# ninocarrillo/pymodem

Hardware: AMD Instinct MI355X
Metric: Msamples/s through demod_chain (higher is better)
Workload: dtype f64+i8

## Files before the change

### include/pymodem_amd.h

```cpp
#ifndef PYMODEM_AMD_H
#define PYMODEM_AMD_H

#include <stddef.h>
#include <stdint.h>

#ifdef __cplusplus
extern "C" {
#endif

#define PM_VERSION 100

typedef enum pm_status {
    PM_OK = 0,
    PM_ERR_HIP = -1,
    PM_ERR_ARG = -2,
    PM_ERR_NODEV = -3,
    PM_ERR_CAPACITY = -4,
    PM_ERR_NOCONVERGE = -5
} pm_status;

typedef struct pm_ctx pm_ctx;

int pm_version(void);
int pm_device_count(void);
// ... 381 lines not shown
    double ms_to_demod_done, ms_to_sliced, ms_to_done;
    double done_at_ms;
} pm_pipe_result;
typedef struct pm_pipe pm_pipe;
int pm_pipe_create(pm_ctx *ctx, const pm_pipe_desc *desc, pm_pipe **out);
int pm_pipe_submit(pm_pipe *pipe, const int16_t *d_audio, int64_t n, int64_t *h_ticket);
int pm_pipe_submit_many(pm_pipe *pipe, const int16_t *const *d_audio, const int64_t *n, int count, int64_t *h_first_ticket);
int pm_pipe_promise(pm_pipe *pipe, int count, int64_t *h_first_ticket);
int pm_pipe_wait(pm_pipe *pipe, int64_t ticket, pm_pipe_result *out);
int pm_pipe_slices(pm_pipe *pipe, int64_t ticket, int chain, const uint8_t **h_data, const int64_t **h_addr, const uint8_t **h_plain, int64_t *h_count);
int pm_pipe_bitmap(pm_pipe *pipe, int64_t ticket, int chain, uint64_t *h_words, int64_t words);
int pm_pipe_slots(pm_pipe *pipe);
int pm_pipe_release(pm_pipe *pipe, int64_t ticket);
int pm_pipe_drain(pm_pipe *pipe);
int pm_pipe_stats(pm_pipe *pipe, int64_t *h_batches, int64_t *h_batch_recordings, double *h_slice_busy_ms, double *h_host_busy_ms);
pm_ctx *pm_pipe_side_ctx(pm_pipe *pipe, int worker);
pm_ctx *pm_pipe_demod_ctx(pm_pipe *pipe, int k);
int pm_pipe_destroy(pm_pipe *pipe);

#ifdef __cplusplus
}
#endif
#endif
```

### pymodem_amd/_native.py

```python
import ctypes
import os

_HERE = os.path.dirname(os.path.abspath(__file__))
_LIB = None


class NativeError(RuntimeError):
    pass


def library_path():
    return os.environ.get("PYMODEM_AMD_LIB") or os.path.join(_HERE, "libpymodem_amd.so")


class AGCParams(ctypes.Structure):
    _fields_ = [(k, ctypes.c_double) for k in ("attack_rate", "decay_rate", "sustain_time", "sample_rate", "target_amplitude")]


class Loop(ctypes.Structure):
    _fields_ = [(k, ctypes.c_double) for k in (
        "phase_scaling", "index_scaling", "set_frequency", "b0", "b1", "a1", "p_rate", "i_rate", "i_limit", "gain",
        "phase", "control", "sine", "cosine", "x0", "x1", "y0", "integral", "proportional",
        "bb0", "bb1", "ba1", "cx0", "cx1", "cy0", "sx0", "sx1", "sy0")]

# ... 270 lines not shown
    "pm_lbatch_tail_ctx": ([_vp], _vp),
    "pm_lbatch_loop_ctx": ([_vp], _vp),
    "pm_lbatch_slice_ctx": ([_vp], _vp),
    "pm_lbatch_destroy": ([_vp], _int),
    "pm_prof_intervals": ([_vp, _int, _vp, _vp, _i64, ctypes.POINTER(_i64)], _int),
    "pm_pipe_create": ([_vp, ctypes.POINTER(PipeDesc), ctypes.POINTER(_vp)], _int),
    "pm_pipe_submit": ([_vp, _vp, _i64, ctypes.POINTER(_i64)], _int),
    "pm_pipe_submit_many": ([_vp, _vp, _vp, _int, _vp], _int),
    "pm_pipe_promise": ([_vp, _int, _vp], _int),
    "pm_pipe_wait": ([_vp, _i64, ctypes.POINTER(PipeResult)], _int),
    "pm_pipe_release": ([_vp, _i64], _int),
    "pm_pipe_slices": ([_vp, _i64, _int, ctypes.POINTER(_vp), ctypes.POINTER(_vp), ctypes.POINTER(_vp), ctypes.POINTER(_i64)], _int),
    "pm_pipe_bitmap": ([_vp, _i64, _int, _vp, _i64], _int),
    "pm_pipe_slots": ([_vp], _int),
    "pm_pipe_drain": ([_vp], _int),
    "pm_pipe_stats": ([_vp, ctypes.POINTER(_i64), ctypes.POINTER(_i64), ctypes.POINTER(ctypes.c_double), ctypes.POINTER(ctypes.c_double)], _int),
    "pm_pipe_side_ctx": ([_vp, _int], _vp),
    "pm_pipe_demod_ctx": ([_vp, _int], _vp),
    "pm_pipe_destroy": ([_vp], _int),
    "pm_costas_bpsk": ([_vp, ctypes.POINTER(Loop), _int, _vp, _vp, _i64, _i64, _vp, _i64], _int),
    "pm_costas_qpsk": ([_vp, ctypes.POINTER(Loop), _int, _vp, _vp, _i64, _i64, _vp, _vp, _i64], _int),
    "pm_pll_afsk": ([_vp, ctypes.POINTER(Loop), _int, _vp, _vp, _i64, _i64, _vp, _i64], _int),
    "pm_mpsk_loop": ([_vp, ctypes.POINTER(Loop), _int, _vp, _vp, _vp, _vp, _i64, _i64, _vp, _vp, _i64], _int),
    "pm_slice_binary": ([_vp, _vp, _i64, ctypes.POINTER(SlicerParams), _vp, _vp, _i64, ctypes.POINTER(_i64)], _int),
    "pm_slice_quadrature": ([_vp, _vp, _vp, _i64, ctypes.POINTER(SlicerParams), _vp, _vp, _i64, ctypes.POINTER(_i64)], _int),
    "pm_slice_batch": ([_vp, ctypes.POINTER(SliceJob), _int], _int),
    "pm_slicer_tune": ([_vp, _i64], _int),
    "pm_slicer_limits": ([_vp, _i64], _int),
    "pm_slice_compact": ([_vp, _vp, _int, _vp, ctypes.c_size_t, ctypes.POINTER(_i64), ctypes.POINTER(ctypes.c_size_t)], _int),
    "pm_stream_scan": ([_vp, ctypes.POINTER(ScanJob), _int, _vp, ctypes.c_size_t, ctypes.POINTER(_i64), ctypes.POINTER(ctypes.c_size_t)], _int),
# ... 69 lines not shown
```

### pymodem_amd/chain_execute.py

```python
import ctypes
from concurrent.futures import ThreadPoolExecutor

import numpy as np

from ._native import Loop, check, lib, quick
from .device import Context, DeviceBuffer
from .modems import AFSKModem, AFSKPLLModem, BPSKModem, MPSKModem, QPSKModem
from .slicer import slice_batch


def process_chain(chain, input_audio):
    demod_audio = chain[1].demod(input_audio)
    sliced_data = chain[2].slice(demod_audio)
    descrambled_data = chain[3].stream_unscramble_8bit(sliced_data)
    return chain[4].decode(descrambled_data)


def multiprocess_chain(chain, input_audio, queue):
    queue.put(process_chain(chain, input_audio))


def process_chain_device(chain, input_audio, stages=None):
    demod_audio = chain[1].demod_signs(input_audio)
    sliced_data = chain[2].slice(demod_audio)
# ... 943 lines not shown
        check(lib().pm_pipe_bitmap(self._h, int(ticket), int(chain), buf.ctypes.data_as(ctypes.c_void_p), max(words, 1)))
        return np.unpackbits(buf.view(np.uint8), bitorder="little")[: int(nout)].astype(bool)

    def release(self, ticket):
        check(lib().pm_pipe_release(self._h, int(ticket)))

    def drain(self):
        check(lib().pm_pipe_drain(self._h))

    def stats(self):
        b, r = ctypes.c_int64(), ctypes.c_int64()
        s, h = ctypes.c_double(), ctypes.c_double()
        check(lib().pm_pipe_stats(self._h, ctypes.byref(b), ctypes.byref(r), ctypes.byref(s), ctypes.byref(h)))
        return {"slice_batches": b.value, "recordings": r.value, "slice_busy_ms": s.value, "host_busy_ms": h.value}

    def side_contexts(self):
        out = []
        for entry, first in ((lib().pm_pipe_side_ctx, 0), (lib().pm_pipe_demod_ctx, 1)):
            i = first
            while True:
                c = entry(self._h, i)
                if not c:
                    break
                out.append(Context.borrowed(c, self._ctx.device))
                i += 1
        return out

    def _destroy(self):
        h, self._h = self._h, None
        if h is not None:
# ... 95 lines not shown
```

### pymodem_amd/csrc/pm_afsk.hip

```cpp
#include "pm_fir_dev.h"
#include "pm_bpf8_dev.h"
#include "pm_afsk_sweep.h"
#include <chrono>
#include <cmath>
#include <cstdlib>
#include <cstring>

namespace {
using namespace pm_sweep;

template <int R, bool VEC, bool SPLIT = false>
__global__ __launch_bounds__(kThreads) void afsk_correlate_kernel(const double *__restrict__ x, int64_t n,
                                                                  const double *__restrict__ mi, const double *__restrict__ mq,
                                                                  const double *__restrict__ si, const double *__restrict__ sq,
                                                                  int m, double *__restrict__ y, int64_t nout, double *__restrict__ y2 = nullptr)
{
    extern __shared__ double xs[];
    constexpr int T = kThreads * R;
    const int t = threadIdx.x;
    const int span = T + m - 1;
    const int64_t tile0 = (int64_t)blockIdx.x * T;
    if (VEC) {
        stage_vec<R>(x, n, tile0, span, t, xs);
    } else {
// ... 161 lines not shown
    for (int i = 0; i < L; ++i) {
        mv[i] = slide_sqrt(a * a + b * b);
        sv[i] = slide_sqrt(c * c + d * d);
        if (i + 1 < L) {
            const double xk = xr[i], xn = xr[slide_slot<L>(i + m)];
            const double a2 = __builtin_fma(T.mr, a, __builtin_fma(-T.ms, b, __builtin_fma(-T.mer, xk, xn)));
            const double b2 = __builtin_fma(T.ms, a, __builtin_fma(T.mr, b, -T.mes * xk));
            const double c2 = __builtin_fma(T.sr, c, __builtin_fma(-T.ss, d, __builtin_fma(-T.ser, xk, xn)));
            const double d2 = __builtin_fma(T.ss, c, __builtin_fma(T.sr, d, -T.ses * xk));
            a = a2; b = b2; c = c2; d = d2;
        }
    }
}

typedef const double __attribute__((address_space(4))) *const_f64_ptr;
template <int L>
__device__ __forceinline__ void slide_run_f32(const double *__restrict__ xs, const double *__restrict__ tp, int run, int m, const SlideTones &T,
                                              float (&mv)[L], float (&sv)[L], const double *tg = nullptr)
{
    const double *xr = xs + run * (L + 1);
    double a = 0.0, b = 0.0, c = 0.0, d = 0.0;
    if (tg) {
        const_f64_ptr tq = (const_f64_ptr)tg;
        const double *xb = xr;
        int i = 0;
        for (; i + L <= m; i += L, xb += L + 1, tq += 4 * L) {
#pragma unroll
            for (int j = 0; j < L; ++j) {
                const double v = xb[j];
                a = __builtin_fma(tq[4 * j + 0], v, a);
                b = __builtin_fma(tq[4 * j + 1], v, b);
                c = __builtin_fma(tq[4 * j + 2], v, c);
                d = __builtin_fma(tq[4 * j + 3], v, d);
            }
        }
        for (int j = 0; i + j < m; ++j) {
            const double v = xb[j];
            a = __builtin_fma(tq[4 * j + 0], v, a);
            b = __builtin_fma(tq[4 * j + 1], v, b);
            c = __builtin_fma(tq[4 * j + 2], v, c);
            d = __builtin_fma(tq[4 * j + 3], v, d);
        }
    } else {
        const double2v *tq = reinterpret_cast<const double2v *>(tp);
        const double *xb = xr;
        int i = 0;
        for (; i + L <= m; i += L, xb += L + 1, tq += 2 * L) {
#pragma unroll
            for (int j = 0; j < L; ++j) {
                const double v = xb[j];
                const double2v h01 = tq[2 * j], h23 = tq[2 * j + 1];
                a = __builtin_fma(h01.x, v, a);
                b = __builtin_fma(h01.y, v, b);
                c = __builtin_fma(h23.x, v, c);
                d = __builtin_fma(h23.y, v, d);
            }
        }
        for (int j = 0; i + j < m; ++j) {
            const double v = xb[j];
            const double2v h01 = tq[2 * j], h23 = tq[2 * j + 1];
            a = __builtin_fma(h01.x, v, a);
            b = __builtin_fma(h01.y, v, b);
            c = __builtin_fma(h23.x, v, c);
            d = __builtin_fma(h23.y, v, d);
        }
    }
#pragma unroll
    for (int i = 0; i < L; ++i) {
        mv[i] = __builtin_amdgcn_sqrtf((float)__builtin_fma(a, a, b * b));
        sv[i] = __builtin_amdgcn_sqrtf((float)__builtin_fma(c, c, d * d));
        if (i + 1 < L) {
            const double xk = xr[i], xn = xr[slide_slot<L>(i + m)];
            const double a2 = __builtin_fma(T.mr, a, __builtin_fma(-T.ms, b, __builtin_fma(-T.mer, xk, xn)));
            const double b2 = __builtin_fma(T.ms, a, __builtin_fma(T.mr, b, -T.mes * xk));
            const double c2 = __builtin_fma(T.sr, c, __builtin_fma(-T.ss, d, __builtin_fma(-T.ser, xk, xn)));
            const double d2 = __builtin_fma(T.ss, c, __builtin_fma(T.sr, d, -T.ses * xk));
            a = a2; b = b2; c = c2; d = d2;
        }
    }
}

// ... 391 lines not shown
#define PM_LPF8_F32MAG 1
#endif

#ifndef PM_LPF8_RECOMB32
#define PM_LPF8_RECOMB32 1
#endif
#ifndef PM_LPF8_WAVES
#define PM_LPF8_WAVES 4
#endif
template <bool ONE>
__device__ __forceinline__ void lpf8_sweep_tile(double *__restrict__ xs, unsigned char *__restrict__ planes, double *__restrict__ tp, int4v *__restrict__ bl,
                                                unsigned *__restrict__ wl, float *__restrict__ wmax8, int sweep, bool lds_ok, int t, int64_t tile0,
                                                const double *__restrict__ mi, const double *__restrict__ mq, const double *__restrict__ ui,
                                                const double *__restrict__ uq, int m, const SlideTones &T, const Lpf8Args &Q, int ml, int64_t nout, int G,
                                                const SweepArgs &P, double E, unsigned long long *__restrict__ list, int *__restrict__ count, int cap,
                                                const double *tg = nullptr)
{
    constexpr int L = kFuseRun, TILE = kThreads * 8;
    const int nmag = TILE + ml - 1, nruns = (nmag + L - 1) / L;
    if (!tg)
        for (int i = t; i < m; i += kThreads) {
            tp[4 * i + 0] = mi[m - 1 - i];
            tp[4 * i + 1] = mq[m - 1 - i];
            tp[4 * i + 2] = ui[m - 1 - i];
            tp[4 * i + 3] = uq[m - 1 - i];
        }
    lds_barrier();
#if PM_LPF8_F32MAG
    float mv[L], sv[L];
    if (t < nruns) slide_run_f32<L>(xs, tp, t, m, T, mv, sv, tg);
    float vmaxf = 0.0f, vsumf = 0.0f;
    if (t < nruns) {
        if (ONE) {
            const float g0 = (float)P.gain[0], ag0 = fabsf(g0);
#pragma unroll
            for (int i = 0; i < L; ++i) {
                vsumf = fmaxf(vsumf, fmaf(ag0, sv[i], mv[i]));
                mv[i] = fmaf(-g0, sv[i], mv[i]);
            }
        }
#pragma unroll
        for (int i = 0; i < L; ++i) vmaxf = fmaxf(vmaxf, ONE ? fabsf(mv[i]) : fmaxf(mv[i], sv[i]));
    }
#pragma unroll
    for (int off = 32; off > 0; off >>= 1) {
// ... 62 lines not shown
                    const double sc = scalable ? __builtin_fma(val[4 * q + i], scale, 6755399441055744.0) : 6755399441055744.0;
                    w[i] = ((unsigned)__double2loint(sc) + 0x808080u) ^ 0x808080u;
#endif
                }
                const unsigned a01 = __builtin_amdgcn_perm(w[1], w[0], 0x05010400u), a23 = __builtin_amdgcn_perm(w[3], w[2], 0x05010400u);
                unsigned char *at = planes + (size_t)stream * kL8Dig * kL8Plane + L * t + 4 * q;
                *reinterpret_cast<unsigned *>(at) = __builtin_amdgcn_perm(a23, a01, 0x05040100u);
                *reinterpret_cast<unsigned *>(at + kL8Plane) = __builtin_amdgcn_perm(a23, a01, 0x07060302u);
                *reinterpret_cast<unsigned *>(at + 2 * kL8Plane) =
                    __builtin_amdgcn_perm(w[1], w[0], 0x0c0c0602u) | __builtin_amdgcn_perm(w[3], w[2], 0x06020c0cu);
            }
        };
        put(mv, 0);
        if (!ONE) put(sv, 1);
    }
    const int lane = t & 63, wave = t >> 6, r = lane & 15, g4 = lane >> 4;
    for (int i = t; i < 2 * kL8Dig * 64; i += kThreads) bl[i] = Q.btab[i];
    lds_barrier();
    const int64_t nout64 = ((nout + 63) >> 6) * 64;
#pragma unroll 1
    for (int q = 0; q < 2; ++q) {
        const int tl = (wave * 2 + q) * 256;
        const int64_t go = tile0 + tl;
        if (go >= nout64) break;
        double a[4], b[4];
#pragma unroll
        for (int stream = 0; stream < (ONE ? 1 : 2); ++stream) {
            int4v acc[kL8Acc];
#pragma unroll
            for (int w = 0; w < kL8Acc; ++w) acc[w] = int4v{0, 0, 0, 0};
// ... 47 lines not shown
            if (uns) {
#pragma unroll
                for (int v = 0; v < 4; ++v)
                    if (16 * v < lim && !(fabs(y[v]) > Ecmp)) {
                        const unsigned mine = lds_ok ? atomicAdd(&wl[kTailCap], 1u) : (unsigned)kTailCap;
                        if (mine < (unsigned)kTailCap) {
                            wl[mine] = ((unsigned)sweep << 20) | ((unsigned)g << 16) | (unsigned)(tl + 64 * g4 + 16 * v + r);
                        } else {
                            const int idx = atomicAdd(count, 1);
                            if (idx < cap) list[idx] = ((unsigned long long)g << 48) | (unsigned long long)(go + 64 * g4 + 16 * v + r);
                        }
                    }
            }
        }
    }
}

template <bool ONE>
__global__ __launch_bounds__(kThreads) __attribute__((amdgpu_waves_per_eu(PM_LPF8_WAVES, PM_LPF8_WAVES))) void afsk_slide_lpf8_kernel(const double *__restrict__ x, int64_t n, const double *__restrict__ mi,
                                                                   const double *__restrict__ mq, const double *__restrict__ ui,
                                                                   const double *__restrict__ uq, int m, SlideTones T, Lpf8Args Q, int ml,
                                                                   int64_t nout, int G, SweepArgs P, double E, unsigned long long *__restrict__ list,
                                                                   int *__restrict__ count, int cap, int region0, SweepTail TL)
{
    extern __shared__ double xs[];
    constexpr int L = kFuseRun, TILE = kThreads * 8;
    const int t = threadIdx.x;
    const int64_t tile0 = (int64_t)blockIdx.x * TILE;
    const int nmag = TILE + ml - 1, nruns = (nmag + L - 1) / L, xspan = nruns * L + m - 1;
    double *tp = xs + region0;
// ... 46 lines not shown
    unsigned long long *list;
    int *count;
    int64_t nout;
};
struct FusedArgs {
    FusedSweep s[2];
    const int16_t *audio;
    int64_t n, nb;
    const pm_bpf8_dev::i4 *bp_btab;
    pm_bpf8_dev::Scales sc;
    SweepSource src;
    int xs_span;
    int aplane;
    int xw_doubles, plane_bytes, mmax;
    int lds_ok, cap;
};

#ifndef PM_FUSED8_WAVES
#define PM_FUSED8_WAVES 5
#endif
template <int KB, bool ONE0, int NS, bool ONE1>
__global__ __launch_bounds__(kThreads) __attribute__((amdgpu_waves_per_eu(PM_FUSED8_WAVES, PM_FUSED8_WAVES))) void afsk_fused8_kernel(FusedArgs A)
{
    extern __shared__ double xs[];
#if defined(PM_FUSED8_PRIO) && PM_FUSED8_PRIO > 0
    __builtin_amdgcn_s_setprio(PM_FUSED8_PRIO);
#endif
    constexpr int L = kFuseRun, TILE = kThreads * 8;
    const int t = threadIdx.x, lane = t & 63, wave = t >> 6;
    const int64_t tile0 = (int64_t)blockIdx.x * TILE;
    unsigned char *const planes = reinterpret_cast<unsigned char *>(xs + A.xw_doubles);
    double *const tp = reinterpret_cast<double *>(planes + A.plane_bytes);
    int4v *const bl = reinterpret_cast<int4v *>(tp + 4 * A.mmax);
    unsigned *const wl = reinterpret_cast<unsigned *>(bl + 2 * kL8Dig * 64);
    float *const wmax8 = reinterpret_cast<float *>(wl + kTailCap + 4);
    if (t == 0) wl[kTailCap] = 0;
    unsigned char *const ap0 = planes, *const ap1 = planes + A.aplane;
    pm_bpf8_dev::stage_planes_rt(A.audio, A.n, tile0, t, kThreads, ap0, ap1, A.aplane);
    {
        lds_barrier();
        const int r = lane & 15, g = lane >> 4;
        const int ntiles = (A.xs_span + 255) >> 8;
        for (int q = wave; q < ntiles; q += kThreads / 64) {
            double val[4];
            const pm_bpf8_dev::i4 *bt = A.bp_btab;
            asm volatile("" : "+s"(bt));
            pm_bpf8_dev::tile_values_tab<KB, 4>(ap0, ap1, bt, q * 256, lane, A.sc, val);
#pragma unroll
            for (int v = 0; v < 4; ++v) {
                const int p = q * 256 + 16 * (4 * g + v) + r;
                if (p < A.xs_span) xs[slide_slot<L>(p)] = tile0 + p < A.nb ? val[v] : 0.0;
            }
        }
    }
    lds_barrier();
    {
        const FusedSweep &S = A.s[0];
        if (tile0 < ((S.nout + 63) >> 6) * 64)
            lpf8_sweep_tile<ONE0>(xs, planes, tp, bl, wl, wmax8, 0, A.lds_ok != 0, t, tile0, S.mi, S.mq, S.ui, S.uq, S.m, S.T, S.Q, S.ml, S.nout, S.G, S.P, S.E,
                                  S.list, S.count, A.cap, S.tg);
    }
    if (NS == 2) {
        lds_barrier();
        const FusedSweep &S = A.s[1];
        if (tile0 < ((S.nout + 63) >> 6) * 64)
            lpf8_sweep_tile<ONE1>(xs, planes, tp, bl, wl, wmax8, 1, A.lds_ok != 0, t, tile0, S.mi, S.mq, S.ui, S.uq, S.m, S.T, S.Q, S.ml, S.nout, S.G, S.P, S.E,
                                  S.list, S.count, A.cap, S.tg);
    }
    __syncthreads();
    const int ne = (int)(wl[kTailCap] < (unsigned)kTailCap ? wl[kTailCap] : (unsigned)kTailCap);
    for (int e = 0; e < ne; ++e) {
        const unsigned ent = wl[e];
        const int g = (int)(ent >> 16) & 15;
        const int64_t k = tile0 + (int64_t)(ent & 0xFFFFu);
        if (NS == 1 || (ent >> 20) == 0) {
            const FusedSweep &S = A.s[0];
            const double *si = S.space + (size_t)g * 2 * S.m;
            sweep_tail_entry<kThreads>(xs, t, nullptr, S.mi, S.mq, si, si + S.m, S.m, S.lpf, S.ml, A.src, k, reinterpret_cast<unsigned long long *>(S.P.bits[g]));
        } else {
            const FusedSweep &S = A.s[1];
            const double *si = S.space + (size_t)g * 2 * S.m;
            sweep_tail_entry<kThreads>(xs, t, nullptr, S.mi, S.mq, si, si + S.m, S.m, S.lpf, S.ml, A.src, k, reinterpret_cast<unsigned long long *>(S.P.bits[g]));
        }
    }
}

__global__ void sweep_mail_reset_kernel(int *__restrict__ count, int *__restrict__ keep, int *__restrict__ mail, int n)
{
    if ((int)threadIdx.x < n) {
        const int c = count[threadIdx.x];
        keep[threadIdx.x] = c;
        mail[threadIdx.x] = c;
        count[threadIdx.x] = 0;
    }
    __threadfence_system();
}

template <bool AUDIO>
__global__ __launch_bounds__(64) void sweep_exact_kernel(const double *__restrict__ x, const double *__restrict__ mi, const double *__restrict__ mq,
// ... 430 lines not shown
    int v = 0;
    PM_HIP(hipMemcpyAsync(&v, ctx->sweep_count, sizeof(int), hipMemcpyDeviceToHost, ctx->stream));
    PM_HIP(hipStreamSynchronize(ctx->stream));
    *h_uncertain = v;
    return PM_OK;
}

int pm_afsk_group_run(pm_ctx *ctx, const int16_t *d_audio, int64_t n, const double *d_bpf, int mb, double *d_bpf_out, double x_bound,
                      const pm_afsk_sweep_desc *h_sweeps, int nsweeps, int64_t *h_tickets)
{
    return pm_afsk_group_run_plan(ctx, d_audio, n, d_bpf, mb, d_bpf_out, x_bound, h_sweeps, nsweeps, h_tickets, nullptr, nullptr);
}

}

static int afsk_group_run_fused(pm_ctx *ctx, const int16_t *d_audio, int64_t n, const double *d_bpf, int mb, double x_bound, const pm_afsk_sweep_desc *h_sweeps,
                                int nsweeps, const pm_bpf8_plan *plan, const pm_lpf8_plan *const *lpf8, const pm_sweep_cells *cells, bool *fused)
{
    *fused = false;
    if (!plan || !lpf8 || !cells || !cells->d_list || nsweeps < 1 || nsweeps > 2 || ctx->tune.afsk_split || ctx->tune.afsk_unfused || ctx->tune.fuse_run == 16 ||
        ((uintptr_t)d_audio & 15) != 0)
        return PM_OK;
    int kb = 0;
    const void *btab = nullptr;
    double sc6[6];
    if (pm_bpf8_plan_view(plan, &kb, &btab, sc6) != PM_OK || (kb != 3 && kb != 4)) return PM_OK;
    FusedArgs A;
    memset(&A, 0, sizeof(A));
    const int64_t nb = n - mb + 1;
    const double e_x = pm_bpf8_error(plan);
    if (!(e_x >= 0.0 && e_x < 1e-6 * x_bound)) return PM_OK;
    SweepShape shape[2];
    for (int k = 0; k < nsweeps; ++k) shape[k] = SweepShape{h_sweeps[k].m, h_sweeps[k].ml, h_sweeps[k].groups == 1};
    const Lpf8Layout Y = lpf8_layout(shape, nsweeps, mb, kb);
    if (!Y.fuses) return PM_OK;
    for (int k = 0; k < nsweeps; ++k) {
        const pm_afsk_sweep_desc &w = h_sweeps[k];
        const pm_lpf8_plan *q = lpf8[k];
        if (!q || !w.h_tones || w.m < 2 || q->ml != w.ml || w.groups < 1 || w.groups > kSweepMax || !w.h_bits || !w.h_gains) return PM_OK;
        if (!(w.h_tones->tap_dev >= 0.0 && w.h_tones->tap_dev < 1e-6) || !(w.lpf_abs_sum > 0.0 && w.lpf_abs_sum < 1e300)) return PM_OK;
        if (nb < (int64_t)w.m + w.ml - 1) return PM_OK;
        FusedSweep &S = A.s[k];
        S.mi = w.d_mark_i; S.mq = w.d_mark_q; S.ui = w.d_unit_i; S.uq = w.d_unit_q;
        S.space = w.d_space; S.lpf = w.d_lpf;
        {
            pm_lpf8_plan *mq_ = const_cast<pm_lpf8_plan *>(q);
            if (!(mq_->d_tpl && mq_->tpl_m == w.m && mq_->tpl_src[0] == w.d_mark_i && mq_->tpl_src[1] == w.d_mark_q && mq_->tpl_src[2] == w.d_unit_i &&
                  mq_->tpl_src[3] == w.d_unit_q)) {
                if (mq_->d_tpl) { PM_HIP(hipStreamSynchronize(ctx->stream)); (void)hipFree(mq_->d_tpl); mq_->d_tpl = nullptr; }
                PM_HIP(hipMalloc(&mq_->d_tpl, sizeof(double) * 4 * (size_t)w.m + 256));
                hipLaunchKernelGGL(pack_templates_kernel, dim3((unsigned)pm_cdiv(4 * (int64_t)w.m, 256)), dim3(256), 0, ctx->stream, w.d_mark_i, w.d_mark_q, w.d_unit_i,
                                   w.d_unit_q, w.m, (double *)mq_->d_tpl);
                PM_HIP(hipGetLastError());
                PM_HIP(hipStreamSynchronize(ctx->stream));
                mq_->tpl_m = w.m;
                mq_->tpl_src[0] = w.d_mark_i; mq_->tpl_src[1] = w.d_mark_q; mq_->tpl_src[2] = w.d_unit_i; mq_->tpl_src[3] = w.d_unit_q;
            }
            S.tg = ctx->tune.sweep_lds_templates ? nullptr : (const double *)mq_->d_tpl;
        }
        S.m = w.m; S.ml = w.ml; S.G = w.groups;
        S.one = w.groups == 1;
        double gmax = 0.0;
        if (!sweep_args(w.h_gains, w.h_bits, w.groups, &S.P, &gmax)) return PM_OK;
        S.T = slide_tones(w.h_tones);
        S.E = sweep_bound(w.m, w.lpf_abs_sum, gmax, x_bound, w.h_tones, kFuseRun, e_x);
        S.Q = lpf8_args(q, gmax, S.one);
        S.list = cells->d_list + (size_t)k * kSweepCap;
        S.count = cells->d_count + k;
        S.nout = nb - w.m - w.ml + 2;
    }
    A.audio = d_audio;
    A.n = n;
    A.nb = nb;
    A.bp_btab = (const pm_bpf8_dev::i4 *)btab;
// ... 2 lines not shown
    A.src = SweepSource{d_audio, d_bpf, mb, e_x};
    A.xs_span = Y.xs_span; A.aplane = Y.aplane; A.mmax = Y.mmax;
    A.xw_doubles = Y.xw_doubles; A.plane_bytes = Y.plane_bytes;
    A.cap = kSweepCap;
    A.lds_ok = Y.lds_ok && !ctx->tune.sweep_no_tail;
    const size_t lds_launch = Y.lds + (size_t)std::max(0, ctx->tune.fused_lds_pad);
    int64_t tiles = 0;
    double bits_out = 0.0, flops = 2.0 * mb * (double)nb;
    for (int k = 0; k < nsweeps; ++k) {
        tiles = std::max(tiles, pm_cdiv(A.s[k].nout, (int64_t)kThreads * 8));
        bits_out += (double)A.s[k].G * (double)A.s[k].nout / 8;
        flops += (4.0 * A.s[k].m / kFuseRun + 18.0) * (double)(nb - A.s[k].m + 1) + (A.s[k].one ? 1.0 : 2.0) * 2.0 * A.s[k].ml * (double)A.s[k].nout +
                 2.0 * A.s[k].G * (double)A.s[k].nout;
    }
    PM_ARG(tiles >= 1 && tiles < (1LL << 31));
    {
        PmProf prof(ctx, PM_K_FIR_F64);
        prof.work((double)n * 2 + bits_out, flops);
        auto go = [&](auto kernel) -> int {
            if (int rc = allow_lds(kernel, lds_launch)) return rc;
            hipLaunchKernelGGL(kernel, dim3((unsigned)tiles), dim3(kThreads), lds_launch, ctx->stream, A);
            return PM_OK;
        };
        int rc = PM_OK;
        const bool o0 = A.s[0].one != 0, o1 = nsweeps == 2 && A.s[1].one != 0;
#define PM_FUSED_GO(KB)                                                                                                             \
        rc = nsweeps == 1 ? (o0 ? go(afsk_fused8_kernel<KB, true, 1, false>) : go(afsk_fused8_kernel<KB, false, 1, false>))              \
                          : (o0 ? (o1 ? go(afsk_fused8_kernel<KB, true, 2, true>) : go(afsk_fused8_kernel<KB, true, 2, false>))          \
                                : (o1 ? go(afsk_fused8_kernel<KB, false, 2, true>) : go(afsk_fused8_kernel<KB, false, 2, false>)));
        if (kb == 3) { PM_FUSED_GO(3) } else { PM_FUSED_GO(4) }
// ... 158 lines not shown
```

### pymodem_amd/csrc/pm_bpf8_dev.h

```cpp
#pragma once
#include <hip/hip_runtime.h>
#include <cstdint>

namespace pm_bpf8_dev {

typedef int i4 __attribute__((ext_vector_type(4)));

struct Scales { double s[5]; double c0; };

__device__ __forceinline__ void stage_planes_rt(const int16_t *__restrict__ x, int64_t n, int64_t wg0, int t, int threads, unsigned char *__restrict__ p0,
                                                unsigned char *__restrict__ p1, int span)
{
    for (int p = t * 8; p < span; p += threads * 8) {
        const int64_t gi = wg0 + p;
        uint32_t d0 = 0, d1 = 0, d2 = 0, d3 = 0;
        if (gi + 8 <= n) {
            const uint4 v = *reinterpret_cast<const uint4 *>(x + gi);
            d0 = v.x; d1 = v.y; d2 = v.z; d3 = v.w;
        } else {
            uint16_t s[8];
#pragma unroll
            for (int q = 0; q < 8; ++q) s[q] = gi + q < n ? (uint16_t)x[gi + q] : (uint16_t)0;
            d0 = s[0] | (uint32_t)s[1] << 16; d1 = s[2] | (uint32_t)s[3] << 16; d2 = s[4] | (uint32_t)s[5] << 16; d3 = s[6] | (uint32_t)s[7] << 16;
        }
// ... 51 lines not shown
#pragma unroll
        for (int b = 0; b < D; ++b) {
            acc[b] = __builtin_amdgcn_mfma_i32_16x16x64_i8(a0, B[b], acc[b], 0, 0, 0);
            acc[b + 1] = __builtin_amdgcn_mfma_i32_16x16x64_i8(a1, B[b], acc[b + 1], 0, 0, 0);
        }
    }
#pragma unroll
    for (int v = 0; v < 4; ++v) {
        double x = sc.c0;
#pragma unroll
        for (int w = 0; w < kWeights; ++w) x = __builtin_fma((double)acc[w][v], sc.s[w], x);
        val[v] = x;
    }
}

}
```

### pymodem_amd/csrc/pm_common.h

```cpp
#pragma once
#include <hip/hip_runtime.h>
#include <cstdarg>
#include <cstdint>
#include <cstdio>
#include <vector>
#include "../../include/pymodem_amd.h"

constexpr size_t PM_PINNED_BYTES = 256 * 1024;
constexpr int kSweepRing = 64;
constexpr int kSweepCap = 65536;

struct pm_sweep_cells {
    int *d_count = nullptr;
    int *h_mail = nullptr;
    unsigned long long *d_list = nullptr;
};

struct pm_tuning {
    int fir_no_short = 0;
    int fuse_run = 0;
    int afsk_unfused = 0;
    int afsk_lpf8 = 0;
    int loop_wide = -1;
    int64_t loop_lds_min = 0;
// ... 98 lines not shown
int pm_bpf8_rows_max(pm_ctx *ctx, const pm_bpf8_plan *p, const int16_t *const *d_rows, int rows, int64_t n, unsigned long long *d_keys, double *d_out,
                     unsigned long long *d_redone = nullptr);
struct pm_lpf8_plan {
    int ml = 0, S = 0, device = 0;
    double tapq_int = 0;
    double qabs = 0;
    double dlow = 0;
    double hmax = 0;
    void *d_btab = nullptr;
    void *d_tpl = nullptr;
    const void *tpl_src[4] = {nullptr, nullptr, nullptr, nullptr};
    int tpl_m = 0;
};
int pm_lpf8_plan_create(pm_ctx *ctx, const double *h_taps, int ml, pm_lpf8_plan **out);
void pm_lpf8_plan_destroy(pm_lpf8_plan *p);
int pm_afsk_group_run_plan(pm_ctx *ctx, const int16_t *d_audio, int64_t n, const double *d_bpf, int mb, double *d_bpf_out, double x_bound,
                           const pm_afsk_sweep_desc *h_sweeps, int nsweeps, int64_t *h_tickets, const pm_bpf8_plan *plan,
                           const pm_lpf8_plan *const *lpf8 = nullptr, const pm_sweep_cells *cells = nullptr);
int pm_afsk_sweep_exact_list(pm_ctx *ctx, const int16_t *d_audio, const double *d_bpf, int mb, const pm_afsk_sweep_desc *w, uint64_t *const *h_bits,
                             const unsigned long long *d_list, const int *d_count);

extern "C" int pm_codec_fetch_batch_clean(pm_codec *const *codecs, const int64_t *counts, int n, pm_packet *h_out, int threads);

struct pm_rowslice;
int pm_rowslice_create(pm_ctx *ctx, const pm_slicer_params *h_params, int chains, pm_rowslice **out);
void pm_rowslice_destroy(pm_rowslice *rs);
bool pm_rowslice_made_for(const pm_rowslice *rs, const pm_slicer_params *h_params, int chains);
int pm_rowslice_chunk(pm_ctx *ctx, const pm_rowslice *rs, int rows, int quad, const uint64_t *d_bi, const uint64_t *d_bq, int64_t stride, int64_t first,
                      int64_t count, pm_rowslice_rec *d_recs, uint8_t *d_data, uint16_t *d_steps, int64_t cap);

// ... 22 lines not shown
```

### pymodem_amd/csrc/pm_pipe.hip

```cpp
#include "pm_common.h"
#include <atomic>
#include <chrono>
#include <condition_variable>
#include <cstring>
#include <deque>
#include <map>
#include <memory>
#include <mutex>
#include <string>
#include <pthread.h>
#include <thread>
#include <vector>

namespace {

constexpr int kMaxChains = 64;
constexpr int kCompactHead = PM_COMPACT_HEAD;

double now_ms()
{
    return std::chrono::duration<double, std::milli>(std::chrono::steady_clock::now().time_since_epoch()).count();
}

struct HostBlock {
// ... 87 lines not shown
    unsigned long long *d_lists = nullptr;
    std::vector<int> free_cells;
    bool keep_slices = false, trace = false;
    bool packets = false;
    bool frames = false;
    bool addrs = false;
    bool scan = false;
    bool host_copy = false;
    bool skip_decode = false;
    int64_t next_ticket = 0, submitted = 0, finished = 0;
    int64_t promised = 0;
    bool promise_failed = false;
    bool closing = false;
    std::vector<std::thread> threads;
    std::atomic<int64_t> batches{0}, batch_recordings{0};
    double busy_slice_ms = 0, busy_host_ms = 0, t_origin = now_ms();
};

namespace {

void rows_clean(RowBlock *b)
{
    for (int64_t k = 0; k < b->used; ++k) {
        pm_packet &q = b->rows[k];
        const int32_t len = k < (int64_t)b->lens.size() ? b->lens[(size_t)k] : PM_PKT_MAX;
        memset(q.data, 0, (size_t)len);
        memset(&q, 0, offsetof(pm_packet, data));
    }
    b->used = 0;
    b->lens.clear();
// ... 162 lines not shown
                    p->slice_q.pop_front();
                }
                if (hipEventSynchronize(nxt->demod_done) != hipSuccess) fail(*nxt, pm_set_error(PM_ERR_HIP, "the demod stage of recording %lld failed", (long long)nxt->ticket));
                nxt->t_ready = now_ms();
                batch.push_back(nxt);
            }
        }
        const double t0 = now_ms();
        const int nch = p->nchains, nb = (int)batch.size();
        int rc = PM_OK;
        std::vector<int> cells_back;
        for (auto &r : batch) {
            if (!p->nsweeps) break;
            std::vector<int64_t> unc(p->nsweeps);
            for (int s = 0; s < p->nsweeps; ++s) unc[s] = ((volatile int *)p->h_cells)[(size_t)r->cell * p->nsweeps + s];
            for (int s = 0; s < p->nsweeps && !r->status; ++s) {
                if (unc[s] <= 0) continue;
                if (unc[s] <= kSweepCap) {
                    if ((rc = pm_afsk_sweep_exact_list(side, r->d_audio, p->d_bpf, p->mb, &p->sweeps[s], p->sweep_bits_store[r->slot][s].data(),
                                                       p->d_lists + ((size_t)r->cell * p->nsweeps + s) * kSweepCap, p->d_cells + (size_t)r->cell * 2 * p->nsweeps + p->nsweeps + s)))
                        fail(*r, rc);
                    continue;
                }
                for (int c = 0; c < nch && !r->status; ++c)
                    if (p->chains[c].sweep == s && (rc = exact_chain(p, side, w, *r, c))) fail(*r, rc);
            }
            cells_back.push_back(r->cell);
            r->cell = -1;
        }
        std::vector<std::pair<int, int>> act;
// ... 456 lines not shown
                if (hipMemcpy(h.data(), d.d_bpf, h.size() * sizeof(double), hipMemcpyDeviceToHost) != hipSuccess)
                    rc = pm_set_error(PM_ERR_HIP, "pm_pipe_create: reading the band-pass taps back failed");
                else
                    rc = pm_bpf8_plan_create(ctx, h.data(), d.mb, &p->bpf8);
            }
        }
        p->lpf8.assign(d.nsweeps, nullptr);
        {
            const char *e = getenv("PM_PIPE_LPF8");
            for (int s = 0; s < d.nsweeps && !rc && !(e && e[0] == '0'); ++s) {
                const pm_afsk_sweep_desc &w = p->sweeps[s];
                if (!p->has_tones[s] || w.ml + 15 > 128 || w.m < 2) continue;
                std::vector<double> h((size_t)w.ml);
                if (hipMemcpy(h.data(), w.d_lpf, h.size() * sizeof(double), hipMemcpyDeviceToHost) != hipSuccess)
                    rc = pm_set_error(PM_ERR_HIP, "pm_pipe_create: reading the low-pass taps back failed");
                else
                    rc = pm_lpf8_plan_create(ctx, h.data(), w.ml, &p->lpf8[s]);
            }
        }
        if (rc) break;
        p->bits_words = (size_t)(d.max_samples + 63) / 64 + 2;
        p->d_bits.assign((size_t)p->slots * d.nchains, nullptr);
        for (size_t i = 0; i < p->d_bits.size() && !rc; ++i) {
            if (!(rc = pm_malloc(ctx, p->bits_words * 8, &q))) p->d_bits[i] = (uint64_t *)q;
        }
        if (rc) break;
        p->sweep_bits_store.resize(p->slots);
        for (int sl = 0; sl < p->slots; ++sl) {
            p->sweep_bits_store[sl].resize(d.nsweeps);
            for (int s = 0; s < d.nsweeps; ++s) {
                p->sweep_bits_store[sl][s].resize(p->sweeps[s].groups);
                for (int g = 0; g < p->sweeps[s].groups; ++g) p->sweep_bits_store[sl][s][g] = p->d_bits[(size_t)sl * d.nchains + seen[s][g]];
// ... 256 lines not shown
    PM_HIP(hipMemcpy(h_words, p->d_bits[(size_t)slot * p->nchains + p->bit_owner[chain]], (size_t)words * 8, hipMemcpyDeviceToHost));
    return PM_OK;
}

int pm_pipe_stats(pm_pipe *p, int64_t *h_batches, int64_t *h_batch_recordings, double *h_slice_busy_ms, double *h_host_busy_ms)
{
    PM_ARG(p != nullptr);
    std::unique_lock<std::mutex> lk(p->mu);
    if (h_batches) *h_batches = p->batches.load();
    if (h_batch_recordings) *h_batch_recordings = p->batch_recordings.load();
    if (h_slice_busy_ms) *h_slice_busy_ms = p->busy_slice_ms;
    if (h_host_busy_ms) *h_host_busy_ms = p->busy_host_ms;
    return PM_OK;
}

pm_ctx *pm_pipe_side_ctx(pm_pipe *p, int worker)
{
    return (p && worker >= 0 && worker < (int)p->side.size()) ? p->side[worker] : nullptr;
}

pm_ctx *pm_pipe_demod_ctx(pm_pipe *p, int k)
{
    return (p && k >= 0 && k < (int)p->demod.size()) ? p->demod[k] : nullptr;
}

}
```

Measured before the change: 284,200.

## Software-pipeline template sums and band-pass MFMA operands, pack templates at pipe creation

The sliding start sums now go through a double-buffered fetch/compute helper that loads the next group of template taps and samples while FMAs run on the current group. The int8 band-pass MFMA loop prefetches the next k-block's weight operands into registers ahead of use. Template packing moves from the per-run fused launch path to pipe creation, which removes a possible allocation and stream sync from the hot path. The change also adds an optional s_memtime phase clock (compiled out by default) and a counter of mailed undecided cells. The prefetching uses more registers, which could lower occupancy.

```diff
diff --git a/include/pymodem_amd.h b/include/pymodem_amd.h
--- a/include/pymodem_amd.h
+++ b/include/pymodem_amd.h
@@ -419,6 +419,7 @@
 int pm_pipe_release(pm_pipe *pipe, int64_t ticket);
 int pm_pipe_drain(pm_pipe *pipe);
 int pm_pipe_stats(pm_pipe *pipe, int64_t *h_batches, int64_t *h_batch_recordings, double *h_slice_busy_ms, double *h_host_busy_ms);
+int pm_pipe_undecided(pm_pipe *pipe, int64_t *h_mailed);
 pm_ctx *pm_pipe_side_ctx(pm_pipe *pipe, int worker);
 pm_ctx *pm_pipe_demod_ctx(pm_pipe *pipe, int k);
 int pm_pipe_destroy(pm_pipe *pipe);
diff --git a/pymodem_amd/_native.py b/pymodem_amd/_native.py
--- a/pymodem_amd/_native.py
+++ b/pymodem_amd/_native.py
@@ -308,6 +308,7 @@
     "pm_pipe_bitmap": ([_vp, _i64, _int, _vp, _i64], _int),
     "pm_pipe_slots": ([_vp], _int),
     "pm_pipe_drain": ([_vp], _int),
+    "pm_pipe_undecided": ([_vp, ctypes.POINTER(_i64)], _int),
     "pm_pipe_stats": ([_vp, ctypes.POINTER(_i64), ctypes.POINTER(_i64), ctypes.POINTER(ctypes.c_double), ctypes.POINTER(ctypes.c_double)], _int),
     "pm_pipe_side_ctx": ([_vp, _int], _vp),
     "pm_pipe_demod_ctx": ([_vp, _int], _vp),
diff --git a/pymodem_amd/chain_execute.py b/pymodem_amd/chain_execute.py
--- a/pymodem_amd/chain_execute.py
+++ b/pymodem_amd/chain_execute.py
@@ -981,6 +981,11 @@
         check(lib().pm_pipe_stats(self._h, ctypes.byref(b), ctypes.byref(r), ctypes.byref(s), ctypes.byref(h)))
         return {"slice_batches": b.value, "recordings": r.value, "slice_busy_ms": s.value, "host_busy_ms": h.value}
 
+    def undecided(self):
+        k = ctypes.c_int64()
+        check(lib().pm_pipe_undecided(self._h, ctypes.byref(k)))
+        return k.value
+
     def side_contexts(self):
         out = []
         for entry, first in ((lib().pm_pipe_side_ctx, 0), (lib().pm_pipe_demod_ctx, 1)):
diff --git a/pymodem_amd/csrc/pm_afsk.hip b/pymodem_amd/csrc/pm_afsk.hip
--- a/pymodem_amd/csrc/pm_afsk.hip
+++ b/pymodem_amd/csrc/pm_afsk.hip
@@ -5,6 +5,7 @@
 #include <cmath>
 #include <cstdlib>
 #include <cstring>
+#include <mutex>
 
 namespace {
 using namespace pm_sweep;
@@ -199,57 +200,99 @@
 }
 
 typedef const double __attribute__((address_space(4))) *const_f64_ptr;
+
+enum { kPhStart, kPhStaged, kPhBandpass, kPhSweep0, kPhTail = kPhSweep0 + 8, kPhStamps };
+#if defined(PM_FUSED8_PHASE_CLOCK) && PM_FUSED8_PHASE_CLOCK
+struct PhaseClock {
+    unsigned long long *row = nullptr;
+    __device__ __forceinline__ void stamp(int k) const
+    {
+        unsigned long long now;
+        __builtin_amdgcn_sched_barrier(0);
+        asm volatile("s_memtime %0\n\ts_waitcnt lgkmcnt(0)" : "=s"(now)::"memory");
+        __builtin_amdgcn_sched_barrier(0);
+        if (row && (threadIdx.x & 63) == 0) row[k] = now;
+    }
+};
+#else
+struct PhaseClock {
+    __device__ __forceinline__ void stamp(int) const {}
+};
+#endif
+
+constexpr int kTplPad = 256;
+template <int L, int TB, bool SC>
+__device__ __forceinline__ void slide_start_sums(const double *__restrict__ xr, const double *__restrict__ tpl, int m, double &a, double &b, double &c, double &d)
+{
+    static_assert(L % TB == 0, "a group lies inside one block of the padded window");
+    static_assert(TB * 4 * 8 <= kTplPad && TB <= L - 1, "the group fetched past the last whole one stays inside the table's padding and the window");
+    const double *xw = xr;
+    int at = 0, q = 0;
+    auto fetch = [&](double (&h)[4 * TB], double (&v)[TB]) {
+        if (SC) {
+            const_f64_ptr tq = (const_f64_ptr)tpl + 4 * at;
+#pragma unroll
+            for (int k = 0; k < 4 * TB; ++k) h[k] = tq[k];
+        } else {
+            const double2v *tq = reinterpret_cast<const double2v *>(tpl) + 2 * at;
+#pragma unroll
+            for (int k = 0; k < 2 * TB; ++k) {
+                const double2v hh = tq[k];
+                h[2 * k] = hh.x;
+                h[2 * k + 1] = hh.y;
+            }
+        }
+#pragma unroll
+        for (int j = 0; j < TB; ++j) v[j] = xw[j];
+        at += TB;
+        xw += TB;
+        if (++q == L / TB) { q = 0; ++xw; }
+    };
+    auto landed = [] {
+        __builtin_amdgcn_sched_barrier(0);
+        __builtin_amdgcn_s_waitcnt(0xC07F);
+        __builtin_amdgcn_sched_barrier(0);
+    };
+    auto taps = [&](const double (&h)[4 * TB], const double (&v)[TB], int count) {
+#pragma unroll
+        for (int j = 0; j < TB; ++j)
+            if (j < count) {
+                a = __builtin_fma(h[4 * j + 0], v[j], a);
+                b = __builtin_fma(h[4 * j + 1], v[j], b);
+                c = __builtin_fma(h[4 * j + 2], v[j], c);
+                d = __builtin_fma(h[4 * j + 3], v[j], d);
+            }
+    };
+    const int ng = m / TB, rem = m - ng * TB;
+    double h0[4 * TB], v0[TB], h1[4 * TB], v1[TB];
+    fetch(h0, v0);
+    int g = 0;
+    for (; g + 2 <= ng; g += 2) {
+        landed(); fetch(h1, v1); taps(h0, v0, TB);
+        landed(); fetch(h0, v0); taps(h1, v1, TB);
+    }
+    if (g < ng) {
+        landed(); fetch(h1, v1); taps(h0, v0, TB);
+        landed(); taps(h1, v1, rem);
+    } else {
+        landed(); taps(h0, v0, rem);
+    }
+}
+
+#ifndef PM_SLIDE_START_TAPS
+#define PM_SLIDE_START_TAPS 4
+#endif
+constexpr int kStartTapsLds = 3;
 template <int L>
 __device__ __forceinline__ void slide_run_f32(const double *__restrict__ xs, const double *__restrict__ tp, int run, int m, const SlideTones &T,
-                                              float (&mv)[L], float (&sv)[L], const double *tg = nullptr)
+                                              float (&mv)[L], float (&sv)[L], const double *tg = nullptr, const PhaseClock &pc = PhaseClock{},
+                                              int ph = 0)
 {
     const double *xr = xs + run * (L + 1);
     double a = 0.0, b = 0.0, c = 0.0, d = 0.0;
-    if (tg) {
-        const_f64_ptr tq = (const_f64_ptr)tg;
-        const double *xb = xr;
-        int i = 0;
-        for (; i + L <= m; i += L, xb += L + 1, tq += 4 * L) {
-#pragma unroll
-            for (int j = 0; j < L; ++j) {
-                const double v = xb[j];
-                a = __builtin_fma(tq[4 * j + 0], v, a);
-                b = __builtin_fma(tq[4 * j + 1], v, b);
-                c = __builtin_fma(tq[4 * j + 2], v, c);
-                d = __builtin_fma(tq[4 * j + 3], v, d);
-            }
-        }
-        for (int j = 0; i + j < m; ++j) {
-            const double v = xb[j];
-            a = __builtin_fma(tq[4 * j + 0], v, a);
-            b = __builtin_fma(tq[4 * j + 1], v, b);
-            c = __builtin_fma(tq[4 * j + 2], v, c);
-            d = __builtin_fma(tq[4 * j + 3], v, d);
-        }
-    } else {
-        const double2v *tq = reinterpret_cast<const double2v *>(tp);
-        const double *xb = xr;
-        int i = 0;
-        for (; i + L <= m; i += L, xb += L + 1, tq += 2 * L) {
-#pragma unroll
-            for (int j = 0; j < L; ++j) {
-                const double v = xb[j];
-                const double2v h01 = tq[2 * j], h23 = tq[2 * j + 1];
-                a = __builtin_fma(h01.x, v, a);
-                b = __builtin_fma(h01.y, v, b);
-                c = __builtin_fma(h23.x, v, c);
-                d = __builtin_fma(h23.y, v, d);
-            }
-        }
-        for (int j = 0; i + j < m; ++j) {
-            const double v = xb[j];
-            const double2v h01 = tq[2 * j], h23 = tq[2 * j + 1];
-            a = __builtin_fma(h01.x, v, a);
-            b = __builtin_fma(h01.y, v, b);
-            c = __builtin_fma(h23.x, v, c);
-            d = __builtin_fma(h23.y, v, d);
-        }
-    }
+    if (tg) slide_start_sums<L, PM_SLIDE_START_TAPS, true>(xr, tg, m, a, b, c, d);
+    else slide_start_sums<L, kStartTapsLds, false>(xr, tp, m, a, b, c, d);
+    pc.stamp(ph);
 #pragma unroll
     for (int i = 0; i < L; ++i) {
         mv[i] = __builtin_amdgcn_sqrtf((float)__builtin_fma(a, a, b * b));
@@ -671,8 +714,9 @@
                                                 const double *__restrict__ mi, const double *__restrict__ mq, const double *__restrict__ ui,
                                                 const double *__restrict__ uq, int m, const SlideTones &T, const Lpf8Args &Q, int ml, int64_t nout, int G,
                                                 const SweepArgs &P, double E, unsigned long long *__restrict__ list, int *__restrict__ count, int cap,
-                                                const double *tg = nullptr)
-{
+                                                const double *tg = nullptr, const PhaseClock &pc = PhaseClock{})
+{
+    const int ph = kPhSweep0 + 4 * sweep;
     constexpr int L = kFuseRun, TILE = kThreads * 8;
     const int nmag = TILE + ml - 1, nruns = (nmag + L - 1) / L;
     if (!tg)
@@ -685,7 +729,9 @@
     lds_barrier();
 #if PM_LPF8_F32MAG
     float mv[L], sv[L];
-    if (t < nruns) slide_run_f32<L>(xs, tp, t, m, T, mv, sv, tg);
+    if (t < nruns) slide_run_f32<L>(xs, tp, t, m, T, mv, sv, tg, pc, ph);
+    else pc.stamp(ph);
+    pc.stamp(ph + 1);
     float vmaxf = 0.0f, vsumf = 0.0f;
     if (t < nruns) {
         if (ONE) {
@@ -778,6 +824,7 @@
         put(mv, 0);
         if (!ONE) put(sv, 1);
     }
+    pc.stamp(ph + 2);
     const int lane = t & 63, wave = t >> 6, r = lane & 15, g4 = lane >> 4;
     for (int i = t; i < 2 * kL8Dig * 64; i += kThreads) bl[i] = Q.btab[i];
     lds_barrier();
@@ -855,6 +902,7 @@
             }
         }
     }
+    pc.stamp(ph + 3);
 }
 
 template <bool ONE>
@@ -931,8 +979,14 @@
     int aplane;
     int xw_doubles, plane_bytes, mmax;
     int lds_ok, cap;
+#if defined(PM_FUSED8_PHASE_CLOCK) && PM_FUSED8_PHASE_CLOCK
+    unsigned long long *clk;
+#endif
 };
 
+#ifndef PM_FUSED8_BPF_AHEAD
+#define PM_FUSED8_BPF_AHEAD 1
+#endif
 #ifndef PM_FUSED8_WAVES
 #define PM_FUSED8_WAVES 5
 #endif
@@ -952,9 +1006,19 @@
     unsigned *const wl = reinterpret_cast<unsigned *>(bl + 2 * kL8Dig * 64);
     float *const wmax8 = reinterpret_cast<float *>(wl + kTailCap + 4);
     if (t == 0) wl[kTailCap] = 0;
+    PhaseClock pc;
+#if defined(PM_FUSED8_PHASE_CLOCK) && PM_FUSED8_PHASE_CLOCK
+    if (A.clk && (blockIdx.x & 63) == 0) pc.row = A.clk + ((size_t)(blockIdx.x >> 6) * (kThreads / 64) + __builtin_amdgcn_readfirstlane(wave)) * kPhStamps;
+#endif
+    pc.stamp(kPhStart);
     unsigned char *const ap0 = planes, *const ap1 = planes + A.aplane;
     pm_bpf8_dev::stage_planes_rt(A.audio, A.n, tile0, t, kThreads, ap0, ap1, A.aplane);
+    pc.stamp(kPhStaged);
     {
+#if PM_FUSED8_BPF_AHEAD
+        pm_bpf8_dev::i4 B[4];
+        pm_bpf8_dev::tile_operands_tab<KB, 4>(A.bp_btab, lane, B);
+#endif
         lds_barrier();
         const int r = lane & 15, g = lane >> 4;
         const int ntiles = (A.xs_span + 255) >> 8;
@@ -962,7 +1026,11 @@
             double val[4];
             const pm_bpf8_dev::i4 *bt = A.bp_btab;
             asm volatile("" : "+s"(bt));
+#if PM_FUSED8_BPF_AHEAD
+            pm_bpf8_dev::tile_values_tab_ahead<KB, 4>(ap0, ap1, bt, q * 256, lane, A.sc, B, val);
+#else
             pm_bpf8_dev::tile_values_tab<KB, 4>(ap0, ap1, bt, q * 256, lane, A.sc, val);
+#endif
 #pragma unroll
             for (int v = 0; v < 4; ++v) {
                 const int p = q * 256 + 16 * (4 * g + v) + r;
@@ -970,19 +1038,20 @@
             }
         }
     }
+    pc.stamp(kPhBandpass);
     lds_barrier();
     {
         const FusedSweep &S = A.s[0];
         if (tile0 < ((S.nout + 63) >> 6) * 64)
             lpf8_sweep_tile<ONE0>(xs, planes, tp, bl, wl, wmax8, 0, A.lds_ok != 0, t, tile0, S.mi, S.mq, S.ui, S.uq, S.m, S.T, S.Q, S.ml, S.nout, S.G, S.P, S.E,
-                                  S.list, S.count, A.cap, S.tg);
+                                  S.list, S.count, A.cap, S.tg, pc);
     }
     if (NS == 2) {
         lds_barrier();
         const FusedSweep &S = A.s[1];
         if (tile0 < ((S.nout + 63) >> 6) * 64)
             lpf8_sweep_tile<ONE1>(xs, planes, tp, bl, wl, wmax8, 1, A.lds_ok != 0, t, tile0, S.mi, S.mq, S.ui, S.uq, S.m, S.T, S.Q, S.ml, S.nout, S.G, S.P, S.E,
-                                  S.list, S.count, A.cap, S.tg);
+                                  S.list, S.count, A.cap, S.tg, pc);
     }
     __syncthreads();
     const int ne = (int)(wl[kTailCap] < (unsigned)kTailCap ? wl[kTailCap] : (unsigned)kTailCap);
@@ -1000,6 +1069,7 @@
             sweep_tail_entry<kThreads>(xs, t, nullptr, S.mi, S.mq, si, si + S.m, S.m, S.lpf, S.ml, A.src, k, reinterpret_cast<unsigned long long *>(S.P.bits[g]));
         }
     }
+    pc.stamp(kPhTail);
 }
 
 __global__ void sweep_mail_reset_kernel(int *__restrict__ count, int *__restrict__ keep, int *__restrict__ mail, int n)
@@ -1460,6 +1530,61 @@
 
 }
 
+int pm_lpf8_plan_set_templates(pm_ctx *ctx, pm_lpf8_plan *q, const double *d_mark_i, const double *d_mark_q, const double *d_unit_i, const double *d_unit_q, int m)
+{
+    PM_CTX(ctx);
+    PM_ARG(q && d_mark_i && d_mark_q && d_unit_i && d_unit_q && m >= 1);
+    if (q->d_tpl) return pm_set_error(PM_ERR_ARG, "pm_lpf8_plan_set_templates: the plan has its templates");
+    PM_HIP(hipMalloc(&q->d_tpl, sizeof(double) * 4 * (size_t)m + kTplPad));
+    hipLaunchKernelGGL(pack_templates_kernel, dim3((unsigned)pm_cdiv(4 * (int64_t)m, 256)), dim3(256), 0, ctx->stream, d_mark_i, d_mark_q, d_unit_i, d_unit_q, m,
+                       (double *)q->d_tpl);
+    PM_HIP(hipGetLastError());
+    PM_HIP(hipStreamSynchronize(ctx->stream));
+    q->tpl_m = m;
+    q->tpl_src[0] = d_mark_i; q->tpl_src[1] = d_mark_q; q->tpl_src[2] = d_unit_i; q->tpl_src[3] = d_unit_q;
+    return PM_OK;
+}
+
+#if defined(PM_FUSED8_PHASE_CLOCK) && PM_FUSED8_PHASE_CLOCK
+static std::mutex g_clk_mu;
+static unsigned long long *g_clk = nullptr;
+static int64_t g_clk_rows[2] = {0, 0}, g_clk_cap = 0;
+static unsigned g_clk_seq = 0;
+static int phase_clock_rows(int64_t tiles, unsigned long long **at)
+{
+    std::lock_guard<std::mutex> lk(g_clk_mu);
+    const int64_t rows = (tiles + 63) / 64;
+    if (rows > g_clk_cap) {
+        if (g_clk) { PM_HIP(hipDeviceSynchronize()); (void)hipFree(g_clk); g_clk = nullptr; g_clk_cap = 0; }
+        const size_t bytes = 2 * (size_t)rows * (kThreads / 64) * kPhStamps * sizeof(unsigned long long);
+        PM_HIP(hipMalloc((void **)&g_clk, bytes));
+        PM_HIP(hipMemset(g_clk, 0, bytes));
+        g_clk_cap = rows;
+    }
+    const int half = (int)(g_clk_seq++ & 1);
+    g_clk_rows[half] = rows;
+    *at = g_clk + (size_t)half * g_clk_cap * (kThreads / 64) * kPhStamps;
+    return PM_OK;
+}
+extern "C" int pm_fused8_phase_clock(unsigned long long *h_words, int64_t cap_words, int64_t *h_rows, int *h_stamps)
+{
+    std::lock_guard<std::mutex> lk(g_clk_mu);
+    PM_ARG(h_words && h_rows && h_stamps);
+    const size_t per = (size_t)(kThreads / 64) * kPhStamps;
+    *h_stamps = kPhStamps;
+    h_rows[0] = g_clk_rows[0]; h_rows[1] = g_clk_rows[1];
+    PM_ARG((int64_t)((g_clk_rows[0] + g_clk_rows[1]) * per) <= cap_words);
+    PM_HIP(hipDeviceSynchronize());
+    size_t at = 0;
+    for (int half = 0; half < 2; ++half) {
+        if (!g_clk_rows[half]) continue;
+        PM_HIP(hipMemcpy(h_words + at, g_clk + (size_t)half * g_clk_cap * per, g_clk_rows[half] * per * sizeof(unsigned long long), hipMemcpyDeviceToHost));
+        at += g_clk_rows[half] * per;
+    }
+    return PM_OK;
+}
+#endif
+
 static int afsk_group_run_fused(pm_ctx *ctx, const int16_t *d_audio, int64_t n, const double *d_bpf, int mb, double x_bound, const pm_afsk_sweep_desc *h_sweeps,
                                 int nsweeps, const pm_bpf8_plan *plan, const pm_lpf8_plan *const *lpf8, const pm_sweep_cells *cells, bool *fused)
 {
@@ -1489,21 +1614,9 @@
         FusedSweep &S = A.s[k];
         S.mi = w.d_mark_i; S.mq = w.d_mark_q; S.ui = w.d_unit_i; S.uq = w.d_unit_q;
         S.space = w.d_space; S.lpf = w.d_lpf;
-        {
-            pm_lpf8_plan *mq_ = const_cast<pm_lpf8_plan *>(q);
-            if (!(mq_->d_tpl && mq_->tpl_m == w.m && mq_->tpl_src[0] == w.d_mark_i && mq_->tpl_src[1] == w.d_mark_q && mq_->tpl_src[2] == w.d_unit_i &&
-                  mq_->tpl_src[3] == w.d_unit_q)) {
-                if (mq_->d_tpl) { PM_HIP(hipStreamSynchronize(ctx->stream)); (void)hipFree(mq_->d_tpl); mq_->d_tpl = nullptr; }
-                PM_HIP(hipMalloc(&mq_->d_tpl, sizeof(double) * 4 * (size_t)w.m + 256));
-                hipLaunchKernelGGL(pack_templates_kernel, dim3((unsigned)pm_cdiv(4 * (int64_t)w.m, 256)), dim3(256), 0, ctx->stream, w.d_mark_i, w.d_mark_q, w.d_unit_i,
-                                   w.d_unit_q, w.m, (double *)mq_->d_tpl);
-                PM_HIP(hipGetLastError());
-                PM_HIP(hipStreamSynchronize(ctx->stream));
-                mq_->tpl_m = w.m;
-                mq_->tpl_src[0] = w.d_mark_i; mq_->tpl_src[1] = w.d_mark_q; mq_->tpl_src[2] = w.d_unit_i; mq_->tpl_src[3] = w.d_unit_q;
-            }
-            S.tg = ctx->tune.sweep_lds_templates ? nullptr : (const double *)mq_->d_tpl;
-        }
+        const bool tabled = q->d_tpl && q->tpl_m == w.m && q->tpl_src[0] == w.d_mark_i && q->tpl_src[1] == w.d_mark_q && q->tpl_src[2] == w.d_unit_i &&
+                            q->tpl_src[3] == w.d_unit_q;
+        S.tg = tabled && !ctx->tune.sweep_lds_templates ? (const double *)q->d_tpl : nullptr;
         S.m = w.m; S.ml = w.ml; S.G = w.groups;
         S.one = w.groups == 1;
         double gmax = 0.0;
@@ -1536,6 +1649,9 @@
                  2.0 * A.s[k].G * (double)A.s[k].nout;
     }
     PM_ARG(tiles >= 1 && tiles < (1LL << 31));
+#if defined(PM_FUSED8_PHASE_CLOCK) && PM_FUSED8_PHASE_CLOCK
+    if (int rc = phase_clock_rows(tiles, &A.clk)) return rc;
+#endif
     {
         PmProf prof(ctx, PM_K_FIR_F64);
         prof.work((double)n * 2 + bits_out, flops);
diff --git a/pymodem_amd/csrc/pm_bpf8_dev.h b/pymodem_amd/csrc/pm_bpf8_dev.h
--- a/pymodem_amd/csrc/pm_bpf8_dev.h
+++ b/pymodem_amd/csrc/pm_bpf8_dev.h
@@ -89,4 +89,52 @@
     }
 }
 
+typedef const i4 __attribute__((address_space(1))) *global_i4_ptr;
+template <int KB, int D>
+__device__ __forceinline__ void tile_operands_tab(const i4 *__restrict__ btab, int lane, i4 (&B)[D])
+{
+    global_i4_ptr bt = (global_i4_ptr)btab;
+#pragma unroll
+    for (int b = 0; b < D; ++b) B[b] = bt[(b * KB) * 64 + lane];
 }
+template <int KB, int D>
+__device__ __forceinline__ void tile_values_tab_ahead(const unsigned char *__restrict__ p0, const unsigned char *__restrict__ p1, const i4 *__restrict__ btab, int tl,
+                                                      int lane, const Scales &sc, i4 (&B)[D], double (&val)[4])
+{
+    constexpr int kWeights = D + 1;
+    global_i4_ptr row[D];
+#pragma unroll
+    for (int b = 0; b < D; ++b) {
+        row[b] = (global_i4_ptr)btab + (b * KB) * 64;
+        asm volatile("" : "+s"(row[b]));
+    }
+    const int r = lane & 15, g = lane >> 4;
+    i4 acc[kWeights];
+#pragma unroll
+    for (int w = 0; w < kWeights; ++w) acc[w] = i4{0, 0, 0, 0};
+#pragma unroll
+    for (int kb = 0; kb < KB; ++kb) {
+        i4 N[D];
+#pragma unroll
+        for (int b = 0; b < D; ++b) N[b] = row[b][(kb + 1 < KB ? kb + 1 : 0) * 64 + lane];
+        const int at = tl + 16 * r + 64 * kb + 16 * g;
+        const i4 a0 = *reinterpret_cast<const i4 *>(p0 + at), a1 = *reinterpret_cast<const i4 *>(p1 + at);
+        __builtin_amdgcn_sched_barrier(0);
+#pragma unroll
+        for (int b = 0; b < D; ++b) {
+            acc[b] = __builtin_amdgcn_mfma_i32_16x16x64_i8(a0, B[b], acc[b], 0, 0, 0);
+            acc[b + 1] = __builtin_amdgcn_mfma_i32_16x16x64_i8(a1, B[b], acc[b + 1], 0, 0, 0);
+        }
+#pragma unroll
+        for (int b = 0; b < D; ++b) B[b] = N[b];
+    }
+#pragma unroll
+    for (int v = 0; v < 4; ++v) {
+        double x = sc.c0;
+#pragma unroll
+        for (int w = 0; w < kWeights; ++w) x = __builtin_fma((double)acc[w][v], sc.s[w], x);
+        val[v] = x;
+    }
+}
+
+}
diff --git a/pymodem_amd/csrc/pm_common.h b/pymodem_amd/csrc/pm_common.h
--- a/pymodem_amd/csrc/pm_common.h
+++ b/pymodem_amd/csrc/pm_common.h
@@ -136,6 +136,7 @@
 };
 int pm_lpf8_plan_create(pm_ctx *ctx, const double *h_taps, int ml, pm_lpf8_plan **out);
 void pm_lpf8_plan_destroy(pm_lpf8_plan *p);
+int pm_lpf8_plan_set_templates(pm_ctx *ctx, pm_lpf8_plan *q, const double *d_mark_i, const double *d_mark_q, const double *d_unit_i, const double *d_unit_q, int m);
 int pm_afsk_group_run_plan(pm_ctx *ctx, const int16_t *d_audio, int64_t n, const double *d_bpf, int mb, double *d_bpf_out, double x_bound,
                            const pm_afsk_sweep_desc *h_sweeps, int nsweeps, int64_t *h_tickets, const pm_bpf8_plan *plan,
                            const pm_lpf8_plan *const *lpf8 = nullptr, const pm_sweep_cells *cells = nullptr);
diff --git a/pymodem_amd/csrc/pm_pipe.hip b/pymodem_amd/csrc/pm_pipe.hip
--- a/pymodem_amd/csrc/pm_pipe.hip
+++ b/pymodem_amd/csrc/pm_pipe.hip
@@ -125,6 +125,7 @@
     bool closing = false;
     std::vector<std::thread> threads;
     std::atomic<int64_t> batches{0}, batch_recordings{0};
+    std::atomic<int64_t> mailed{0};
     double busy_slice_ms = 0, busy_host_ms = 0, t_origin = now_ms();
 };
 
@@ -317,6 +318,7 @@
             if (!p->nsweeps) break;
             std::vector<int64_t> unc(p->nsweeps);
             for (int s = 0; s < p->nsweeps; ++s) unc[s] = ((volatile int *)p->h_cells)[(size_t)r->cell * p->nsweeps + s];
+            for (int s = 0; s < p->nsweeps; ++s) p->mailed += std::max<int64_t>(unc[s], 0);
             for (int s = 0; s < p->nsweeps && !r->status; ++s) {
                 if (unc[s] <= 0) continue;
                 if (unc[s] <= kSweepCap) {
@@ -803,8 +805,8 @@
                 std::vector<double> h((size_t)w.ml);
                 if (hipMemcpy(h.data(), w.d_lpf, h.size() * sizeof(double), hipMemcpyDeviceToHost) != hipSuccess)
                     rc = pm_set_error(PM_ERR_HIP, "pm_pipe_create: reading the low-pass taps back failed");
-                else
-                    rc = pm_lpf8_plan_create(ctx, h.data(), w.ml, &p->lpf8[s]);
+                else if (!(rc = pm_lpf8_plan_create(ctx, h.data(), w.ml, &p->lpf8[s])))
+                    rc = pm_lpf8_plan_set_templates(ctx, p->lpf8[s], w.d_mark_i, w.d_mark_q, w.d_unit_i, w.d_unit_q, w.m);
             }
         }
         if (rc) break;
@@ -1091,6 +1093,13 @@
     return PM_OK;
 }
 
+int pm_pipe_undecided(pm_pipe *p, int64_t *h_mailed)
+{
+    PM_ARG(p != nullptr && h_mailed != nullptr);
+    *h_mailed = p->mailed.load();
+    return PM_OK;
+}
+
 pm_ctx *pm_pipe_side_ctx(pm_pipe *p, int worker)
 {
     return (p && worker >= 0 && worker < (int)p->side.size()) ? p->side[worker] : nullptr;
```

Result: slower. 274,600 (-3.4%).
